# lalithsuresh/rapid

Hardware: NVIDIA H100
Metric: alert_cells_per_sec_to_converged_cut (higher is better)
Workload: dtype u16

## Files before the change

rapid_b200/csrc/cd_bucketed.cu:

```cuda
#include <cooperative_groups.h>

#include <algorithm>
#include <climits>
#include <cstdlib>

#include "cd_internal.cuh"

namespace cg = cooperative_groups;

namespace rapid {

#ifndef RAPID_UNI_MINBLOCKS
#define RAPID_UNI_MINBLOCKS 5
#endif
#ifndef RAPID_SPLIT_LOOP
#define RAPID_SPLIT_LOOP 0
#endif
#ifndef RAPID_PF
#define RAPID_PF 2
#endif
#ifndef RAPID_INVAL_SPLIT
#define RAPID_INVAL_SPLIT 1
#endif
#ifndef RAPID_PF_L1
#define RAPID_PF_L1 0
#endif
#if RAPID_PF_L1
#define RAPID_PF_ASM "prefetch.global.L1 [%0];"
#else
#define RAPID_PF_ASM "prefetch.global.L2 [%0];"
#endif
#ifndef RAPID_MEMO
#define RAPID_MEMO 1
#endif

constexpr int TILE_R = 1024;
constexpr int UNI_THREADS = 128;
constexpr int GEN_THREADS = 256;
constexpr int STAGE = 32;
constexpr int MAXK = RAPID_MAX_K;
constexpr int SMALL_SEG = 4;
constexpr uint32_t T32_NONE = 0xFFFFFFFFu;
constexpr uint64_t T64_NONE = ~0ULL;
constexpr uint32_t RF_K3 = 16u;
constexpr uint32_t RF_ACTIVE = 32u;
constexpr uint32_t RF_MIXED_EMIT = 64u;

constexpr uint32_t MX_ON = 1u, MX_NEG = 2u, MX_HAS_E = 4u, MX_DONE = 8u;
constexpr uint32_t MX_REF = 32u;
constexpr uint32_t MX_TIME = 16u;

constexpr uint32_t PF_SEEN = 1u;
constexpr uint32_t PF_NEGINF = 2u;

struct ChunkAcc {
    uint32_t nL, nH, tp, nUn, fl, minTH, minTLun, pad_;
    uint64_t h1, h2;
    uint32_t nLp, nHp, tpc, minBHp, minBLlong, pad2_;
    uint64_t h1p, h2p;
};

constexpr int PF_SHIFT = 30;
constexpr uint32_t TP_MASK = (1u << PF_SHIFT) - 1u;

struct Partials {
    uint4* cnt;
    uint4* cntp;
    uint64_t* minTH;
    uint64_t* minTLun;
    uint64_t* h1;
    uint64_t* h2;
    uint64_t* h1p;
    uint64_t* h2p;
    uint2* seq;
    int32_t* flag;
    ChunkAcc* chunk;
    int n_tiles;
};

struct Bucketed {
    DevBuf<int32_t> sidx;
    DevBuf<int32_t> seg_cnt, batch_slots;
    DevBuf<int32_t> bins, ovf, cell_batch;
    DevBuf<SubjDesc> desc;
    DevBuf<SubjWalk> walk;
    DevBuf<uint8_t> s_ring, s_status;
    DevBuf<int32_t> p_flag;
    DevBuf<ChunkAcc> p_chunk;
    DevBuf<uint4> p_cnt, p_cntp;
    DevBuf<uint64_t> p_minTH, p_minTLun, p_h1, p_h2, p_h1p, p_h2p;
    DevBuf<uint2> p_seq;
    DevBuf<SubjWalk> pwalk;
    DevBuf<unsigned char> ra_dev;
    DevBuf<uint32_t> mx_fl;
    DevBuf<uint64_t> mx_a, mx_cand, mx_emax;
    DevBuf<uint64_t> mx_p1, mx_p2;
    DevBuf<int32_t> mx_pc;
    DevBuf<unsigned long long> mx_e1, mx_e2;
    DevBuf<int32_t> mx_ec;
    DevBuf<uint64_t> estar;
    DevBuf<int32_t> mx_changed;
    DevBuf<uint32_t> mx_dev;
    DevBuf<int32_t> batch_index;
#if RAPID_INVAL_SPLIT
    DevBuf<int32_t> inv_res, inv_ticket;
    DevBuf<unsigned long long> inv_h1, inv_h2;
#endif
    DevBuf<int32_t> wl_slots, wl_count, wl_listed, wl_so_tab;
    DevBuf<uint8_t> wl_in_tile;
    DevBuf<uint8_t> has_so;
    size_t in_list_slots = 0;
    int n_tiles = 0;
    size_t part_cap = 0;
    int slots_uniform = 0, slots_generic = 0;
    int resolve_grid = 0;
};

struct Visit {
    int c0, c1;
    bool crossL, crossH;
    uint32_t tL, tH;
};

__device__ __forceinline__ Visit visit_uniform(uint32_t ur, const SubjDesc& d, const SubjWalk& w, int L, int H) {
    Visit v;
    v.tL = 0; v.tH = 0;
    if (ur == d.pmask) {
        v.c0 = __popc(ur); v.c1 = __popc(ur | d.bmask);
        v.tL = d.tLf; v.tH = d.tHf;
    } else {
        int c = __popc(ur);
        v.c0 = c;
        const int nr = d.nr;
        for (int q = 0; q < nr; ++q) {
            const int k = w.ring[q];
            const bool isnew = !((ur >> k) & 1u);
            c += isnew;
            if (isnew && c == L) v.tL = w.time[q];
            if (isnew && c == H) v.tH = w.time[q];
        }
        v.c1 = c;
    }
    v.crossL = v.c0 < L && v.c1 >= L;
    v.crossH = v.c0 < H && v.c1 >= H;
    return v;
}

__device__ __forceinline__ Visit visit_counts(uint32_t ur, const SubjDesc& d, uint32_t RM, int L, int H) {
    Visit v;
    v.tL = 0; v.tH = 0;
    v.c0 = __popc(ur);
    v.c1 = __popc((ur | d.bmask) & RM);
    v.crossL = v.c0 < L && v.c1 >= L;
    v.crossH = v.c0 < H && v.c1 >= H;
    return v;
}

struct Acc {
    uint32_t nL = 0, nH = 0, tp = 0, nUn = 0, flags = 0;
    uint32_t minTH = T32_NONE, minTLun = T32_NONE;
    uint64_t h1 = 0, h2 = 0;
    uint32_t nLp = 0, nHp = 0, tpc = 0, minBHp = T32_NONE, minBLlong = T32_NONE;
    uint64_t h1p = 0, h2p = 0;
};

__device__ __forceinline__ bool accumulate(Acc& a, const Visit& v, const SubjDesc& d, int L, int H) {
    if (v.c0 >= L && v.c0 < H) a.tp++;
    if (v.crossL) a.nL++;
    if (v.crossH) { a.nH++; a.minTH = min(a.minTH, v.tH); a.h1 += d.mix1; a.h2 += d.mix2; }
    if (v.c1 >= L && v.c1 < H) {
        if (v.crossL) { a.nUn++; a.minTLun = min(a.minTLun, v.tL); }
        else a.flags |= PF_NEGINF;
        return true;
    }
    return false;
}
// ... 684 lines not shown
    uint64_t* mx_p1;
    uint64_t* mx_p2;
    int32_t* mx_pc;
    uint64_t* estar;
    unsigned long long* mx_e1;
    unsigned long long* mx_e2;
    int32_t* mx_ec;
    int32_t* mx_changed;
    uint32_t* mx_dev;
    const int32_t* slot_of;
    const int32_t* obs;
    const int32_t* touch;
    const int32_t* batch_index;
    int32_t serial;
#if RAPID_INVAL_SPLIT
    int inv_split;
    int32_t* inv_res;
    unsigned long long* inv_h1;
    unsigned long long* inv_h2;
    int32_t* inv_ticket;
#endif
};

__device__ __forceinline__ int32_t block_sum_i32(int32_t v, int32_t* s_red) {
    __syncthreads();
#pragma unroll
    for (int o = 16; o > 0; o >>= 1) v += __shfl_down_sync(0xffffffffu, v, o);
    if ((threadIdx.x & 31) == 0) s_red[threadIdx.x >> 5] = v;
    __syncthreads();
    int32_t s = 0;
    for (int w = 0; w < (int)(blockDim.x >> 5); ++w) s += s_red[w];
    return s;
}

__device__ __forceinline__ void reduce_fresh(const ResolveArgs& a, ChunkAcc* s_fresh, int* s_fhave) {
    const ApplyArgs& ap = a.ap;
    if (threadIdx.x < 32) {
        uint32_t nL = 0, nH = 0, tp = 0, nUn = 0, fl = 0, mTH = T32_NONE, mTL = T32_NONE;
        uint64_t h1 = 0, h2 = 0;
        uint32_t nLp = 0, nHp = 0, tpc = 0, mBH = T32_NONE, mBL = T32_NONE;
        uint64_t h1p = 0, h2p = 0;
        for (int c = threadIdx.x; c < a.n_chunks; c += 32) {
            const ChunkAcc k = ap.part.chunk[c];
            nL += k.nL; nH += k.nH; tp += k.tp; nUn += k.nUn; fl |= k.fl;
            if (k.nH) mTH = min(mTH, k.minTH);
            if (k.nUn) mTL = min(mTL, k.minTLun);
            h1 += k.h1; h2 += k.h2;
            if (a.seq) {
                nLp += k.nLp; nHp += k.nHp; tpc += k.tpc; mBH = min(mBH, k.minBHp); mBL = min(mBL, k.minBLlong);
                h1p += k.h1p; h2p += k.h2p;
            }
        }
#pragma unroll
        for (int o = 16; o > 0; o >>= 1) {
            nL += __shfl_down_sync(0xffffffffu, nL, o); nH += __shfl_down_sync(0xffffffffu, nH, o);
            tp += __shfl_down_sync(0xffffffffu, tp, o);
            nUn += __shfl_down_sync(0xffffffffu, nUn, o); fl |= __shfl_down_sync(0xffffffffu, fl, o);
            mTH = min(mTH, __shfl_down_sync(0xffffffffu, mTH, o)); mTL = min(mTL, __shfl_down_sync(0xffffffffu, mTL, o));
            h1 += __shfl_down_sync(0xffffffffu, h1, o); h2 += __shfl_down_sync(0xffffffffu, h2, o);
            nLp += __shfl_down_sync(0xffffffffu, nLp, o); nHp += __shfl_down_sync(0xffffffffu, nHp, o);
            tpc += __shfl_down_sync(0xffffffffu, tpc, o);
            mBH = min(mBH, __shfl_down_sync(0xffffffffu, mBH, o)); mBL = min(mBL, __shfl_down_sync(0xffffffffu, mBL, o));
            h1p += __shfl_down_sync(0xffffffffu, h1p, o); h2p += __shfl_down_sync(0xffffffffu, h2p, o);
        }
        if (threadIdx.x == 0) {
            ChunkAcc f;
            f.nL = nL; f.nH = nH; f.tp = tp; f.nUn = nUn; f.fl = fl; f.minTH = mTH; f.minTLun = mTL; f.pad_ = 0; f.h1 = h1; f.h2 = h2;
            f.nLp = nLp; f.nHp = nHp; f.tpc = tpc; f.minBHp = mBH; f.minBLlong = mBL; f.pad2_ = 0; f.h1p = h1p; f.h2p = h2p;
            *s_fresh = f;
            *s_fhave = (nH ? 1 : 0) | (nUn ? 2 : 0);
        }
    }
    __syncthreads();
}

__device__ void phase_finalize1(const ResolveArgs& a, int32_t* s_red) {
    const ApplyArgs& ap = a.ap;
    const int any_down = a.bc->any_down;
    __shared__ ChunkAcc s_fresh;
    __shared__ int s_fhave;
    reduce_fresh(a, &s_fresh, &s_fhave);
    int32_t my_mixed = 0, my_times = 0;
    for (int64_t r = (int64_t)blockIdx.x * blockDim.x + threadIdx.x; r < ap.R; r += (int64_t)gridDim.x * blockDim.x) {
        a.mx_fl[r] = 0;
        uint32_t flags = a.rflags[r] & ~(RF_ANN_NOW | RF_K3 | RF_ACTIVE | RF_PRE_DOWN);
        if (flags & RF_SEEN_DOWN) flags |= RF_PRE_DOWN;
        a.out_h1[r] = 0; a.out_h2[r] = 0; a.out_len[r] = 0;
        const bool active = !(flags & RF_ANNOUNCED) && !((ap.dl.flags & RAPID_DELIVERY_BLOCKED) && ap.dl.blocked[r]);
        if (!active) { a.rflags[r] = flags; a.out_ann[r] = (flags & RF_ANNOUNCED) ? 1 : 0; continue; }
        flags |= RF_ACTIVE;
        uint32_t nL = s_fresh.nL, nH = s_fresh.nH, tp = s_fresh.tp, nUn = s_fresh.nUn, fl = s_fresh.fl;
        uint64_t minTH = s_fresh.minTH, minTLun = s_fresh.minTLun, h1 = s_fresh.h1, h2 = s_fresh.h2;
        uint32_t nLp = s_fresh.nLp, nHp = s_fresh.nHp;
        uint64_t h1p = s_fresh.h1p, h2p = s_fresh.h2p;
        bool haveTH = s_fhave & 1, haveTL = (s_fhave & 2) != 0;
        const int tile = (int)(r / TILE_R);
        for (int c0 = 0; c0 < a.n_chunks; c0 += 4) {
            int on[4];
#pragma unroll
            for (int q = 0; q < 4; ++q) on[q] = c0 + q < a.n_chunks ? ap.part.flag[(size_t)(c0 + q) * ap.part.n_tiles + tile] : 0;
            uint4 q4[4], p4[4];
            uint64_t th[4], tl[4], a1[4], a2[4], b1[4], b2[4];
#pragma unroll
            for (int q = 0; q < 4; ++q) {
                if (!on[q]) continue;
                const size_t p = (size_t)(c0 + q) * ap.Rpad + (size_t)r;
                q4[q] = ap.part.cnt[p]; a1[q] = ap.part.h1[p]; a2[q] = ap.part.h2[p];
                if (!a.counts_only) { th[q] = ap.part.minTH[p]; tl[q] = ap.part.minTLun[p]; }
                if (a.seq) { p4[q] = ap.part.cntp[p]; b1[q] = ap.part.h1p[p]; b2[q] = ap.part.h2p[p]; }
            }
#pragma unroll
            for (int q = 0; q < 4; ++q) {
                if (!on[q]) continue;
                const uint32_t cH = q4[q].y, cUn = q4[q].w;
                nL += q4[q].x; nH += cH; tp += q4[q].z & TP_MASK; nUn += cUn; fl |= q4[q].z >> PF_SHIFT;
                if (!a.counts_only) {
                    if (cH && (!haveTH || th[q] < minTH)) { minTH = th[q]; haveTH = true; }
                    if (cUn && (!haveTL || tl[q] < minTLun)) { minTLun = tl[q]; haveTL = true; }
                }
                h1 += a1[q]; h2 += a2[q];
                if (a.seq) { nLp += p4[q].x; nHp += p4[q].y; h1p += b1[q]; h2p += b2[q]; }
            }
        }
        if ((a.uniform || a.counts_only) ? any_down : (fl & PF_SEEN)) flags |= RF_SEEN_DOWN;
        const int32_t npre_old = a.n_pre[r] + (int32_t)nLp - (int32_t)nHp;
        const int32_t npre_new = npre_old + (int32_t)nL - (int32_t)nH;
        const uint64_t p1_old = a.pend_h1[r] + h1p, p2_old = a.pend_h2[r] + h2p;
        const int32_t pc_old = a.pend_cnt[r] + (int32_t)nHp;
        uint64_t ph1 = p1_old + h1, ph2 = p2_old + h2;
        int32_t pc = pc_old + (int32_t)nH;
        const int32_t untouched_pre = npre_old - (int32_t)tp;
        if (nH > 0 && npre_new == 0) {
            a.out_h1[r] = ph1; a.out_h2[r] = ph2; a.out_len[r] = pc;
            ph1 = 0; ph2 = 0; pc = 0;
            flags |= RF_ANNOUNCED | RF_ANN_NOW | RF_RULE_GE_H;
        } else if (nH > 0 && untouched_pre <= 0 && !(fl & PF_NEGINF)) {
            if (a.counts_only) {
                ++my_times;
                a.mx_fl[r] = MX_TIME;
                a.mx_a[r] = T64_NONE; a.mx_cand[r] = T64_NONE; a.mx_emax[r] = 0;
                a.mx_p1[r] = p1_old; a.mx_p2[r] = p2_old; a.mx_pc[r] = pc_old;
            } else if (!(haveTL && minTLun < minTH)) {
                ++my_mixed;
                atomicMin(&a.bc->mx_first, (int32_t)r);
                a.mx_fl[r] = MX_ON;
                a.mx_a[r] = minTLun; a.mx_cand[r] = T64_NONE; a.mx_emax[r] = 0;
                a.mx_p1[r] = p1_old; a.mx_p2[r] = p2_old; a.mx_pc[r] = pc_old;
            }
        }
        if (npre_new > 0 && (flags & RF_SEEN_DOWN)) flags |= RF_K3;
        a.n_pre[r] = npre_new;
        a.pend_h1[r] = ph1; a.pend_h2[r] = ph2; a.pend_cnt[r] = pc;
        a.rflags[r] = flags;
    }
    const int32_t bm = block_sum_i32(my_mixed, s_red), bt = block_sum_i32(my_times, s_red);
    if (threadIdx.x == 0) {
        if (bm) atomicAdd(&a.bc->n_mixed, bm);
        if (bt) atomicAdd(&a.bc->n_times, bt);
    }
}

struct IVisit { int c0, c1; bool crossL, crossH; uint64_t tL, tH; };

__device__ __forceinline__ IVisit interval_visit(const ApplyArgs& a, int uniform, uint32_t ur, const SubjDesc& d, const SubjWalk* w,
                                                 int64_t r, uint64_t rs) {
    IVisit o;
    if (uniform) {
        const Visit v = visit_uniform(ur, d, *w, a.L, a.H);
        o.c0 = v.c0; o.c1 = v.c1; o.crossL = v.crossL; o.crossH = v.crossH; o.tL = v.tL; o.tH = v.tH;
    } else {
        const GVisit v = visit_generic(ur, d, a.sidx, a.s_ring, a.s_status, a.dl, r, rs, a.L, a.H);
        o.c0 = v.c0; o.c1 = v.c1; o.crossL = v.crossL; o.crossH = v.crossH; o.tL = v.tL; o.tH = v.tH;
    }
    return o;
}

struct PassSmem {
    SubjDesc sd[STAGE];
    SubjWalk sw[STAGE];
    const uint8_t* s_old[STAGE];
};

template <int MODE>
__device__ __noinline__ void mixed_pass(const ResolveArgs& m, PassSmem& sm, const int Sb, const int S_before, const int64_t only_r = -1) {
    const ApplyArgs& a = m.ap;
    const int t = threadIdx.x;
    const uint32_t RM = (1u << a.K) - 1u;
    const int L = a.L, H = a.H;
    const int rblocks = (int)(a.Rpad / GEN_THREADS);
    int mchunks = max(1, min((Sb + STAGE - 1) / STAGE, (2 * (int)gridDim.x + rblocks - 1) / rblocks));
    const int mchunk = max(1, (Sb + mchunks - 1) / mchunks);
    mchunks = (Sb + mchunk - 1) / mchunk;
    const int64_t items = (int64_t)rblocks * mchunks;
    for (int64_t wi = blockIdx.x; wi < items; wi += gridDim.x) {
        const int rb = (int)(wi % rblocks), chunk = (int)(wi / rblocks);
        const int64_t r = (int64_t)rb * GEN_THREADS + t;
        const uint32_t fl = r < a.R ? m.mx_fl[r] : 0u;
        const bool on = (only_r < 0 || r == only_r) &&
                        (MODE == 0 ? ((fl & MX_ON) && !(fl & MX_DONE)) : MODE == 1 ? ((fl & MX_DONE) && (fl & MX_HAS_E) && !(fl & MX_REF)) : ((fl & MX_TIME) != 0));
        if (!__syncthreads_or(on ? 1 : 0)) continue;
        const uint64_t ref = on ? (MODE == 0 ? m.mx_a[r] : MODE == 1 ? m.estar[r] : 0ull) : 0ull;
        const uint64_t rs = splitmix64(a.dl.perm_seed + (uint64_t)(a.rbegin + r));
        const int s0 = chunk * mchunk, s1 = min(Sb, s0 + mchunk);
        uint64_t cand = T64_NONE, emax = 0, h1 = 0, h2 = 0, mTH = T64_NONE, mTL = T64_NONE;
        bool neg = false, has_e = false;
        int cnt = 0;
        for (int base = s0; base < s1; base += STAGE) {
            const int n = min(STAGE, s1 - base);
            __syncthreads();
            if (t < n) {
                const SubjDesc d = a.desc[base + t];
// ... 78 lines not shown
        const int32_t oc = a.mx_pc[r] + a.mx_ec[r];
        a.out_h1[r] = o1; a.out_h2[r] = o2; a.out_len[r] = oc;
        a.pend_h1[r] -= o1; a.pend_h2[r] -= o2; a.pend_cnt[r] -= oc;
        a.mx_e1[r] = 0; a.mx_e2[r] = 0; a.mx_ec[r] = 0;
        a.rflags[r] = (a.rflags[r] | RF_ANNOUNCED | RF_ANN_NOW | RF_MIXED_EMIT) & ~RF_RULE_GE_H;
    }
}

__device__ __noinline__ bool emitted_in_batch(const ResolveArgs& e, int32_t s, int64_t r, uint32_t w_new, uint64_t rs) {
    const ApplyArgs& a = e.ap;
    const uint32_t RM = (1u << a.K) - 1u;
    if (e.touch[s] != e.serial) return __popc(w_new & RM) >= a.H && !e.trans.test(s, r);
    const int b = e.batch_index[s];
    const SubjDesc d = a.desc[b];
    const uint32_t old = seq_state(a, d, b, r, (s >= a.bc->S_before ? 0u : a.rows.get(a.rows.alt_lo(s), r)) & RM, true, true);
    if (__popc(old & RM) >= a.H) return true;
    SubjWalk wl;
    if (e.uniform) wl = a.walk[b];
    const IVisit v = interval_visit(a, e.uniform, old & RM, d, &wl, r, rs);
    return v.crossH && v.tH <= e.estar[r];
}

constexpr int INV_STAGE = 128;
struct InvSmem {
    uint8_t* row[INV_STAGE];
    uint64_t mix1[INV_STAGE], mix2[INV_STAGE];
    uint8_t ne[INV_STAGE];
    const uint8_t* e_row[INV_STAGE * MAXK];
    int32_t e_so[INV_STAGE * MAXK];
    uint8_t e_k[INV_STAGE * MAXK];
    uint8_t flag[INV_STAGE];
    uint8_t dense[INV_STAGE];
    int32_t n_dense;
};

template <bool MX>
__device__ void phase_inval_finalize2(const ResolveArgs& e, int mixed, InvSmem& sm, int32_t* s_red) {
    static_assert(TILE_R == 4 * GEN_THREADS, "a thread owns 4 receivers of a tile");
    const ApplyArgs& a = e.ap;
    const uint32_t RM = (1u << a.K) - 1u;
    const int t = threadIdx.x;
    const int n_list = min(*(volatile int32_t*)a.wl.count, a.wl.cap);
    int32_t my_inval = 0;
#if RAPID_INVAL_SPLIT
    const int P = MX ? 1 : max(1, e.inv_split);
    __shared__ int s_fin;
#else
    constexpr int P = 1;
#endif
    for (int tb = blockIdx.x; tb < a.n_tiles * P; tb += gridDim.x) {
        const int tile = P > 1 ? tb % a.n_tiles : tb;
        int lo = 0, hi = n_list;
        if (P > 1) {
            const int per = max(8, (n_list + P - 1) / P);
            lo = min(n_list, (tb / a.n_tiles) * per); hi = min(n_list, lo + per);
        }
        const int64_t rb = (int64_t)tile * TILE_R + (int64_t)t * 4;
        const uint4 rf4 = *reinterpret_cast<const uint4*>(e.rflags + rb);
        uint32_t flags[4] = {rf4.x, rf4.y, rf4.z, rf4.w};
        bool k3[4];
        bool any_k3 = false;
        bool mine[4];
#pragma unroll
        for (int j = 0; j < 4; ++j) {
            mine[j] = rb + j < a.R && (((flags[j] & RF_MIXED_EMIT) != 0 && mixed) == MX);
            k3[j] = mine[j] && (flags[j] & RF_ACTIVE) && (flags[j] & RF_K3);
            any_k3 |= k3[j];
        }
        int32_t res[4] = {0, 0, 0, 0};
        uint64_t kh1[4] = {0, 0, 0, 0}, kh2[4] = {0, 0, 0, 0};
        if (n_list > 0 && __syncthreads_or(any_k3 ? 1 : 0)) {
            for (int base = lo; base < hi; base += INV_STAGE) {
                const int n = min(INV_STAGE, hi - base);
                __syncthreads();
                if (t == 0) sm.n_dense = 0;
                __syncthreads();
                if (t < n) {
                    const int32_t sl = a.wl.slots[base + t];
                    const uint8_t fl = a.wl.in_tile[(size_t)sl * a.wl.n_tiles + tile];
                    sm.flag[t] = fl;
                    sm.row[t] = a.rows.cur_lo(sl);
                    const int32_t subject = a.slot_subject[sl];
                    sm.mix1[t] = fp_mix1(subject); sm.mix2[t] = fp_mix2(subject);
                    int ne = 0;
                    for (int k = 0; k < a.K; ++k) {
                        const int32_t s2 = a.wl.so_tab[(size_t)sl * SO_STRIDE + k];
                        if (s2 < 0) continue;
                        sm.e_row[t * MAXK + ne] = a.rows.cur_lo(s2);
                        sm.e_so[t * MAXK + ne] = s2; sm.e_k[t * MAXK + ne] = (uint8_t)k;
                        ++ne;
                    }
                    sm.ne[t] = (uint8_t)ne;
                    if (fl) sm.dense[atomicAdd(&sm.n_dense, 1)] = (uint8_t)t;
                }
                __syncthreads();
                if (!any_k3) continue;
                const int nd = sm.n_dense;
                for (int g = 0; g < nd; g += 4) {
                    int idx[4];
                    uint2 w2v[4], e0v[4], e1v[4];
#pragma unroll
                    for (int q = 0; q < 4; ++q) {
                        idx[q] = g + q < nd ? (int)sm.dense[g + q] : -1;
                        w2v[q] = make_uint2(0xFFFFFFFFu, 0xFFFFFFFFu); e0v[q] = make_uint2(0u, 0u); e1v[q] = make_uint2(0u, 0u);
                        if (idx[q] < 0) continue;
                        w2v[q] = a.rows.load4(sm.row[idx[q]], rb);
                        const int eb = idx[q] * MAXK, ne = sm.ne[idx[q]];
                        if (ne > 0) e0v[q] = a.rows.load4(sm.e_row[eb], rb);
                        if (ne > 1) e1v[q] = a.rows.load4(sm.e_row[eb + 1], rb);
                    }
#pragma unroll
                    for (int q = 0; q < 4; ++q) {
                        const int i = idx[q];
                        if (i < 0) continue;
                        const int eb = i * MAXK, ee = eb + sm.ne[i];
                        uint32_t w[4];
#pragma unroll
                        for (int j = 0; j < 4; ++j) w[j] = a.rows.word4(w2v[q], j);
                        uint32_t miss[4];
                        uint32_t anymiss = 0;
#pragma unroll
                        for (int j = 0; j < 4; ++j) {
                            const int c = __popc(w[j] & RM);
                            miss[j] = (k3[j] && c >= a.L && c < a.H) ? (~w[j] & RM) : 0u;
                            anymiss |= miss[j];
                        }
                        if (!anymiss) continue;
                        uint32_t implicit[4] = {0u, 0u, 0u, 0u};
                        for (int ei = eb; ei < ee; ++ei) {
                            const int k = sm.e_k[ei];
                            if (!((anymiss >> k) & 1u)) continue;
                            const uint2 o2 = ei == eb ? e0v[q] : ei == eb + 1 ? e1v[q] : a.rows.load4(sm.e_row[ei], rb);
                            uint32_t wo[4];
#pragma unroll
                            for (int j = 0; j < 4; ++j) wo[j] = a.rows.word4(o2, j);
#pragma unroll
                            for (int j = 0; j < 4; ++j) {
                                if (!((miss[j] >> k) & 1u)) continue;
                                if (__popc(wo[j] & RM) < a.L) continue;
                                if (MX) {
                                    const int64_t r = rb + j;
                                    if (emitted_in_batch(e, sm.e_so[ei], r, wo[j], splitmix64(a.dl.perm_seed + (uint64_t)(a.rbegin + r)))) continue;
                                }
                                implicit[j] |= 1u << k;
                            }
                        }
                        bool any = false;
                        uint32_t trans = 0;
#pragma unroll
                        for (int j = 0; j < 4; ++j) {
                            if (!implicit[j]) continue;
                            any = true;
                            w[j] |= implicit[j];
                            const bool raised = __popc(w[j] & RM) >= a.H;
                            if (raised && mixed) trans |= 1u << j;
                            if (raised) { ++res[j]; kh1[j] += sm.mix1[i]; kh2[j] += sm.mix2[i]; }
                        }
                        if (trans) atomicOr(e.trans.word(a.wl.slots[base + i], rb), trans << (rb & 31));
                        if (any) a.rows.store4(sm.row[i], rb, w);
                    }
                }
            }
        }
#if RAPID_INVAL_SPLIT
        if (P > 1) {
#pragma unroll
            for (int j = 0; j < 4; ++j)
                if (res[j] > 0) { atomicAdd(&e.inv_res[rb + j], res[j]); atomicAdd(&e.inv_h1[rb + j], (unsigned long long)kh1[j]); atomicAdd(&e.inv_h2[rb + j], (unsigned long long)kh2[j]); }
            __threadfence();
            __syncthreads();
// ... 88 lines not shown
    __shared__ int s_last;
    __syncthreads();
    if (threadIdx.x == 0) {
        __threadfence();
        s_last = atomicAdd(&a.bc->ticket, 1) == (int)gridDim.x - 1;
    }
    __syncthreads();
    if (!s_last || threadIdx.x != 0) return;
    __threadfence();
    volatile BatchCounts* b = a.bc;
    BatchCounts c;
    c.n_slots = b->n_slots; c.n_valid = b->n_valid; c.n_batch_subj = b->n_batch_subj; c.any_down = b->any_down;
    c.bad_ring = b->bad_ring; c.bad_dst = b->bad_dst; c.n_mixed = b->n_mixed; c.n_inval = b->n_inval; c.S_before = b->S_before;
    c.overflow = b->overflow; c.need_slots = b->need_slots; c.n_times = b->n_times; c.mixed_iters = b->mixed_iters;
    c.n_pairs = *(volatile int32_t*)a.ap.wl.count; c.ticket = 0; c.serial = serial;
    c.seq_last = b->seq_last; c.seq_down = b->seq_down; c.seq_abort = b->seq_abort; c.seq_a1 = b->seq_a1; c.seq_a2 = b->seq_a2;
    c.mx_first = b->mx_first; c.mx_left = b->mx_left;
    if (c.seq_abort) { c.n_slots = c.S_before; b->n_slots = c.S_before; }
    c.sticky_bad_ring = b->sticky_bad_ring | (c.bad_ring >= 0 ? 1 : 0);
    c.sticky_bad_dst = b->sticky_bad_dst | (c.bad_dst >= 0 ? 1 : 0);
    c.sticky_overflow = b->sticky_overflow | (c.overflow ? 1 : 0);
    b->sticky_bad_ring = c.sticky_bad_ring; b->sticky_bad_dst = c.sticky_bad_dst; b->sticky_overflow = c.sticky_overflow;
    *a.snap = c;
    b->n_valid = 0; b->n_batch_subj = 0; b->any_down = 0; b->bad_ring = -1; b->bad_dst = -1; b->n_mixed = 0; b->n_inval = 0;
    b->overflow = 0; b->need_slots = 0; b->n_times = 0; b->mixed_iters = 0; b->ticket = 0;
    b->seq_last = 0; b->seq_down = INT_MAX; b->seq_abort = 0; b->seq_a1 = 0; b->seq_a2 = 0; b->mx_first = INT_MAX; b->mx_left = 0;
    b->S_before = c.n_slots;
}

__device__ void phase_ref_compare(const ResolveArgs& e, const int64_t r0, const int Sb, const int S_before) {
    static_assert(TILE_R == 4 * GEN_THREADS, "a thread owns 4 receivers of a tile");
    const ApplyArgs& a = e.ap;
    const uint32_t RM = (1u << a.K) - 1u;
    const int t = threadIdx.x;
    constexpr int CH = 64;
    __shared__ const uint8_t* s_row[CH];
    __shared__ uint32_t s_ref[CH];
    const int nch = (Sb + CH - 1) / CH;
    const int64_t items = (int64_t)a.n_tiles * nch;
    for (int64_t wi = blockIdx.x; wi < items; wi += gridDim.x) {
        const int tile = (int)(wi % a.n_tiles), ch = (int)(wi / a.n_tiles);
        const int64_t rb = (int64_t)tile * TILE_R + (int64_t)t * 4;
        const int b0 = ch * CH, nb = min(Sb, b0 + CH) - b0;
        __syncthreads();
        if (t < nb) {
            const int32_t slot = a.desc[b0 + t].slot;
            const uint8_t* row = slot >= S_before ? nullptr : a.rows.cur_lo(slot);
            s_row[t] = row;
            s_ref[t] = row ? a.rows.get(row, r0) & RM : 0u;
        }
        __syncthreads();
        uint32_t bits = 0;
#pragma unroll 8
        for (int i = 0; i < nb; ++i) {
            const uint8_t* row = s_row[i];
            if (row == nullptr) continue;
            const uint2 g = a.rows.load4(row, rb);
#pragma unroll
            for (int j = 0; j < 4; ++j) bits |= ((a.rows.word4(g, j) ^ s_ref[i]) & RM) ? 1u << j : 0u;
        }
        if (bits) atomicOr(&e.mx_dev[rb >> 5], bits << (rb & 31));
    }
}
__device__ void phase_ref_adopt(const ResolveArgs& a, const int64_t r0, int32_t* s_red) {
    const uint32_t f0 = a.mx_fl[r0];
    int32_t my = 0;
    for (int64_t r = (int64_t)blockIdx.x * blockDim.x + threadIdx.x; r < a.ap.R; r += (int64_t)gridDim.x * blockDim.x) {
        const uint32_t fl = a.mx_fl[r];
        const bool dev = (a.mx_dev[r >> 5] >> (r & 31)) & 1u;
        if (r != r0 && (fl & MX_ON) && !(fl & MX_DONE)) {
            if (!dev) {
                a.mx_fl[r] = f0 ? (f0 | MX_REF) : 0u;
                if ((f0 & MX_DONE) && (f0 & MX_HAS_E)) { a.estar[r] = a.estar[r0]; a.mx_e1[r] = a.mx_e1[r0]; a.mx_e2[r] = a.mx_e2[r0]; a.mx_ec[r] = a.mx_ec[r0]; }
            } else {
                ++my;
            }
        }
    }
    const int32_t b = block_sum_i32(my, s_red);
    if (threadIdx.x == 0 && b) atomicAdd(&a.bc->mx_left, b);
    if (blockIdx.x == 0 && threadIdx.x == 0 && f0) a.mx_fl[r0] = f0 | MX_REF;
}

__global__ void __launch_bounds__(GEN_THREADS) k_seq_check(const ResolveArgs* __restrict__ ga) {
    const ResolveArgs& a = *ga;
    const ApplyArgs& ap = a.ap;
    __shared__ int32_t s_red[GEN_THREADS / 32];
    __shared__ ChunkAcc s_fresh;
    __shared__ int s_fhave;
    if (a.bc->overflow) return;
    const int64_t r = (int64_t)blockIdx.x * GEN_THREADS + threadIdx.x;
    const uint32_t rf = r < ap.R ? a.rflags[r] : RF_ANNOUNCED;
    const bool active = r < ap.R && !(rf & RF_ANNOUNCED) && !((ap.dl.flags & RAPID_DELIVERY_BLOCKED) && ap.dl.blocked[r]);
    int32_t bad = 0;
    if (blockIdx.y == 0) {
        reduce_fresh(a, &s_fresh, &s_fhave);
        if (active) {
            uint32_t tpc = s_fresh.tpc, mBH = s_fresh.minBHp, mBL = s_fresh.minBLlong;
            const int tile = (int)(r / TILE_R);
            for (int c = 0; c < a.n_chunks; ++c) {
                if (!ap.part.flag[(size_t)c * ap.part.n_tiles + tile]) continue;
                const size_t p = (size_t)c * ap.Rpad + (size_t)r;
                tpc += ap.part.cntp[p].z;
                const uint2 q = ap.part.seq[p];
                mBH = min(mBH, q.x); mBL = min(mBL, q.y);
            }
            const bool ok = mBH == T32_NONE || (a.n_pre[r] - (int32_t)tpc) > 0 || mBL < mBH;
            if (!ok) bad = 1;
        }
    } else {
        const int32_t S = a.bc->n_slots, S_before = a.bc->S_before;
        const uint32_t last = (uint32_t)a.bc->seq_last;
        const int nchunks = (int)gridDim.y - 1;
        const int per = (S + nchunks - 1) / nchunks;
        const int32_t q0 = min(S, ((int)blockIdx.y - 1) * per), q1 = min(S, q0 + per);
        const uint32_t RM = (1u << ap.K) - 1u;
        const uint32_t bDown = receiver_down_batch(ap, rf, false);
        for (int32_t sl = q0; sl < q1; ++sl) {
            if (sl >= S_before || !ap.wl.has_so[sl] || a.touch[sl] == a.serial) continue;
            if (!active || bDown == T32_NONE) continue;
            const uint32_t us = ap.rows.get(sl, r) & RM;
            const int cs = __popc(us);
            if (cs < ap.L || cs >= ap.H) continue;
            for (int k = 0; k < ap.K; ++k) {
                const int32_t so = ap.wl.so_tab[(size_t)sl * SO_STRIDE + k];
                if (so < 0 || ((us >> k) & 1u)) continue;
                const bool o_touched = a.touch[so] == a.serial;
                const int bo_idx = o_touched ? a.batch_index[so] : 0;
                const uint32_t uo = so < S_before ? (ap.rows.get(so, r) & RM) : 0u;
                const uint32_t bLo = observer_L_batch(uo, o_touched ? &ap.desc[bo_idx] : nullptr, o_touched ? &ap.pwalk[bo_idx] : nullptr, ap.L);
                if (bLo != T32_NONE && max(bLo, bDown) <= last) bad = 1;
            }
        }
    }
    const int32_t b = block_sum_i32(bad, s_red);
    if (threadIdx.x == 0 && b) { atomicAdd(&a.bc->seq_abort, b); atomicAdd(blockIdx.y == 0 ? &a.bc->seq_a1 : &a.bc->seq_a2, b); }
}

__global__ void __launch_bounds__(GEN_THREADS) k_finalize1(const ResolveArgs* __restrict__ ga) {
    const ResolveArgs& a = *ga;
    __shared__ int32_t s_red[GEN_THREADS / 32];
    if (a.bc->overflow || a.bc->seq_abort) return;
    phase_finalize1(a, s_red);
}

__global__ void __launch_bounds__(GEN_THREADS, 2) k_mixed_flip(const ResolveArgs* __restrict__ ga) {
    const ResolveArgs& a = *ga;
    cg::grid_group grid = cg::this_grid();
    __shared__ PassSmem sm;
    __shared__ int32_t s_red[GEN_THREADS / 32];
    if (a.bc->overflow || a.bc->seq_abort) return;
    const int Sb = a.bc->n_batch_subj, S_before = a.bc->S_before;
    if (a.counts_only && a.bc->n_times > 0 && Sb > 0) {
        mixed_pass<2>(a, sm, Sb, S_before);
        grid.sync();
        phase_classify_moments(a, s_red);
        grid.sync();
    }
    const int mixed = *(volatile int32_t*)&a.bc->n_mixed > 0 ? 1 : 0;
    if (mixed && Sb > 0) {
        auto analyse = [&](const int64_t only_r) -> int {
            int it = 0;
            for (;; ++it) {
                mixed_pass<0>(a, sm, Sb, S_before, only_r);
                grid.sync();
                if (blockIdx.x == 0 && threadIdx.x == 0) a.mx_changed[(it + 2) & 3] = 0;
                phase_mixed_update(a, &a.mx_changed[it & 3], s_red, only_r);
                grid.sync();
                if (*(volatile int32_t*)&a.mx_changed[it & 3] == 0 || it > Sb + 1) break;
            }
            mixed_pass<1>(a, sm, Sb, S_before, only_r);
            grid.sync();
            if (blockIdx.x == 0 && threadIdx.x == 0) { a.mx_changed[0] = 0; a.mx_changed[1] = 0; a.mx_changed[2] = 0; a.mx_changed[3] = 0; }
            grid.sync();
            return it + 1;
        };
        int iters = 0;
        int left = 1;
        if (a.uniform && !a.ap.seq) {
            const int64_t r0 = (int64_t)*(volatile int32_t*)&a.bc->mx_first;
            iters = analyse(r0);
            phase_ref_compare(a, r0, Sb, S_before);
            grid.sync();
            phase_ref_adopt(a, r0, s_red);
            grid.sync();
            left = *(volatile int32_t*)&a.bc->mx_left;
            for (int64_t q = (int64_t)blockIdx.x * blockDim.x + threadIdx.x; q < (int64_t)(a.ap.Rpad >> 5); q += (int64_t)gridDim.x * blockDim.x) a.mx_dev[q] = 0;
        }
        if (left > 0) iters += analyse(-1);
        if (blockIdx.x == 0 && threadIdx.x == 0) a.bc->mixed_iters = iters;
        phase_mixed_commit(a);
        grid.sync();
    }
    for (int b = blockIdx.x * blockDim.x + threadIdx.x; b < Sb; b += gridDim.x * blockDim.x) a.cur_w[a.ap.desc[b].slot] ^= 1;
}

__global__ void __launch_bounds__(GEN_THREADS, 2) k_inval_finalize2(const ResolveArgs* __restrict__ ga) {
    const ResolveArgs& a = *ga;
    __shared__ InvSmem sm;
    __shared__ int32_t s_red[GEN_THREADS / 32];
    const int mixed = a.bc->n_mixed > 0 ? 1 : 0;
    if (!a.bc->overflow && !a.bc->seq_abort) phase_inval_finalize2<false>(a, mixed, sm, s_red);
    if (a.bc->seq_abort) {
        const int32_t s0 = a.bc->S_before, s1 = a.bc->n_slots;
        for (int32_t sl = s0 + blockIdx.x * blockDim.x + threadIdx.x; sl < s1; sl += gridDim.x * blockDim.x)
            const_cast<int32_t*>(a.slot_of)[a.ap.slot_subject[sl]] = -1;
    }
    if (!mixed) resolve_tail(a, a.serial);
}

__global__ void __launch_bounds__(GEN_THREADS, 2) k_marks(const ResolveArgs* __restrict__ ga) {
    const ResolveArgs& a = *ga;
    cg::grid_group grid = cg::this_grid();
    __shared__ InvSmem sm;
    __shared__ int32_t s_red[GEN_THREADS / 32];
    if (a.bc->n_mixed <= 0) return;
    phase_inval_finalize2<true>(a, 1, sm, s_red);
    grid.sync();
    if (*(volatile int32_t*)&a.bc->n_inval > 0) {
        phase_mixed_mark(a, *(volatile int32_t*)&a.bc->n_slots);
        grid.sync();
    }
    phase_inval_unmark(a);
    resolve_tail(a, a.serial);
}

static Bucketed* state(CD* cd) {
    if (!cd->bucketed_state) cd->bucketed_state = new Bucketed();
    return static_cast<Bucketed*>(cd->bucketed_state);
}

void bucketed_destroy(CD* cd) {
    if (cd->bucketed_state) { delete static_cast<Bucketed*>(cd->bucketed_state); cd->bucketed_state = nullptr; }
}

static WorkList worklist(const Bucketed* b) {
    WorkList wl;
    wl.has_so = b->has_so.p; wl.so_tab = b->wl_so_tab.p; wl.in_tile = b->wl_in_tile.p; wl.listed = b->wl_listed.p;
    wl.slots = b->wl_slots.p; wl.count = b->wl_count.p;
    wl.cap = (int32_t)std::min<size_t>(b->in_list_slots, 0x7fffffff); wl.n_tiles = b->n_tiles;
    return wl;
}

template <typename T>
static int32_t grow_keep(DevBuf<T>& buf, size_t n_old, size_t n_new, cudaStream_t s) {
    DevBuf<T> nb;
    RAPID_CHECK(nb.reserve(std::max<size_t>(n_new, 1)));
    RAPID_CUDA(cudaMemsetAsync(nb.p, 0, std::max<size_t>(n_new, 1) * sizeof(T), s));
    if (n_old && buf.p) RAPID_CUDA(cudaMemcpyAsync(nb.p, buf.p, n_old * sizeof(T), cudaMemcpyDeviceToDevice, s));
    RAPID_CUDA(cudaStreamSynchronize(s));
    std::swap(buf.p, nb.p); std::swap(buf.cap, nb.cap);
    return RAPID_OK;
}

static int32_t ensure_pre_capacity(CD* cd, Bucketed* b) {
    const size_t slots = cd->S_cap;
    if (slots <= b->in_list_slots) return RAPID_OK;
    const size_t o = b->in_list_slots, nt = (size_t)b->n_tiles;
    RAPID_CHECK(grow_keep(b->wl_in_tile, o * nt, slots * nt, cd->stream));
    RAPID_CHECK(grow_keep(b->wl_listed, o, slots, cd->stream));
    RAPID_CHECK(grow_keep(b->wl_slots, o, slots, cd->stream));
    RAPID_CHECK(grow_keep(b->wl_so_tab, o * SO_STRIDE, slots * SO_STRIDE, cd->stream));
    RAPID_CHECK(grow_keep(b->has_so, o, slots, cd->stream));
    b->in_list_slots = slots;
    return RAPID_OK;
}

int32_t bucketed_prep_buffers(CD* cd, int64_t A, PrepOut* po) {
    Bucketed* b = state(cd);
    b->n_tiles = (int)(cd->Rpad / TILE_R);
    RAPID_CHECK(ensure_pre_capacity(cd, b));
    const size_t a = (size_t)std::max<int64_t>(A, 1);
    RAPID_CHECK(b->desc.reserve(a)); RAPID_CHECK(b->walk.reserve(a)); RAPID_CHECK(b->pwalk.reserve(a));
    RAPID_CHECK(b->sidx.reserve(a)); RAPID_CHECK(b->s_ring.reserve(a)); RAPID_CHECK(b->s_status.reserve(a));
    const size_t slots = std::max<size_t>(cd->S_cap, 1);
    RAPID_CHECK(b->batch_index.reserve(slots));
    RAPID_CHECK(b->batch_slots.reserve(slots));
    RAPID_CHECK(b->bins.reserve(slots * 64));
    RAPID_CHECK(b->ovf.reserve(a)); RAPID_CHECK(b->cell_batch.reserve(a));
    if (slots > b->seg_cnt.cap) {
        RAPID_CHECK(b->seg_cnt.reserve(slots));
        RAPID_CUDA(cudaMemsetAsync(b->seg_cnt.p, 0, b->seg_cnt.cap * sizeof(int32_t), cd->stream));
    }
    po->desc = b->desc.p; po->walk = b->walk.p; po->sidx = b->sidx.p; po->s_ring = b->s_ring.p; po->s_status = b->s_status.p;
    po->batch_index = b->batch_index.p; po->seg_cnt = b->seg_cnt.p; po->batch_slots = b->batch_slots.p;
    po->bins = b->bins.p; po->ovf = b->ovf.p; po->pwalk = b->pwalk.p; po->cell_batch = b->cell_batch.p;
    po->wl = worklist(b);
    return RAPID_OK;
}

__global__ void k_clear_sticky(BatchCounts* bc) { bc->sticky_bad_ring = 0; bc->sticky_bad_dst = 0; bc->sticky_overflow = 0; }

int32_t bucketed_clear_sticky(CD* cd) {
    k_clear_sticky<<<1, 1, 0, cd->stream>>>(cd->counts.p);
    RAPID_KERNEL_CHECK();
// ... 121 lines not shown
            const double f = w - std::floor(w);
            double eff;
            if (w <= 1.0) eff = 0.85 + 0.15 * w;
            else eff = w / (std::floor(w) + (f > 0 ? std::max(f, 0.6) : 0.0));
            eff -= 0.001 * cc;
            if (eff > best) { best = eff; n_chunks = cc; }
        }
        if (const char* ov = getenv("RAPID_B200_CHUNKS")) n_chunks = std::max(1, std::min(Sb, atoi(ov)));
    }
    cd->last_chunks = n_chunks;
    const size_t pn = (size_t)n_chunks * cd->Rpad;
    RAPID_CHECK(b->p_cnt.reserve(pn)); RAPID_CHECK(b->p_minTH.reserve(pn)); RAPID_CHECK(b->p_minTLun.reserve(pn));
    RAPID_CHECK(b->p_h1.reserve(pn)); RAPID_CHECK(b->p_h2.reserve(pn));
    if (seq) {
        RAPID_CHECK(b->p_cntp.reserve(pn)); RAPID_CHECK(b->p_h1p.reserve(pn)); RAPID_CHECK(b->p_h2p.reserve(pn));
        RAPID_CHECK(b->p_seq.reserve(pn));
    }
    RAPID_CHECK(b->mx_fl.reserve(cd->Rpad)); RAPID_CHECK(b->mx_a.reserve(cd->Rpad)); RAPID_CHECK(b->mx_cand.reserve(cd->Rpad));
    RAPID_CHECK(b->mx_emax.reserve(cd->Rpad)); RAPID_CHECK(b->mx_p1.reserve(cd->Rpad)); RAPID_CHECK(b->mx_p2.reserve(cd->Rpad));
    RAPID_CHECK(b->mx_pc.reserve(cd->Rpad)); RAPID_CHECK(b->estar.reserve(cd->Rpad));
    if (!b->mx_dev.p || b->mx_dev.cap < (cd->Rpad >> 5)) {
        RAPID_CHECK(b->mx_dev.reserve(std::max<size_t>(cd->Rpad >> 5, 1)));
        RAPID_CUDA(cudaMemsetAsync(b->mx_dev.p, 0, std::max<size_t>(cd->Rpad >> 5, 1) * sizeof(uint32_t), s));
    }
    if (!b->mx_e1.p) {
        RAPID_CHECK(b->mx_e1.reserve(cd->Rpad)); RAPID_CHECK(b->mx_e2.reserve(cd->Rpad)); RAPID_CHECK(b->mx_ec.reserve(cd->Rpad));
        RAPID_CUDA(cudaMemsetAsync(b->mx_e1.p, 0, cd->Rpad * sizeof(unsigned long long), s));
        RAPID_CUDA(cudaMemsetAsync(b->mx_e2.p, 0, cd->Rpad * sizeof(unsigned long long), s));
        RAPID_CUDA(cudaMemsetAsync(b->mx_ec.p, 0, cd->Rpad * sizeof(int32_t), s));
    }
    RAPID_CHECK(b->p_flag.reserve((size_t)n_chunks * std::max(b->n_tiles, 1)));
    RAPID_CHECK(b->p_chunk.reserve((size_t)n_chunks));
    Partials part{b->p_cnt.p, b->p_cntp.p, b->p_minTH.p, b->p_minTLun.p, b->p_h1.p, b->p_h2.p, b->p_h1p.p, b->p_h2p.p, b->p_seq.p, b->p_flag.p, b->p_chunk.p, b->n_tiles};

    ApplyArgs ap;
    ap.rows = RowRef{cd->masks.p, cd->cur.p, cd->Rpad, cd->row_stride, cd->nbuf, cd->hb}; ap.Rpad = cd->Rpad;
    ap.K = cd->K; ap.H = cd->H; ap.L = cd->L; ap.R = cd->R; ap.rbegin = cd->rbegin;
    ap.rflags = cd->rflags.p; ap.dl = dl; ap.bc = cd->counts.p;
    ap.desc = b->desc.p; ap.walk = b->walk.p; ap.pwalk = b->pwalk.p; ap.slot_subject = cd->slot_subject.p;
    ap.touch = cd->touch.p; ap.batch_index = b->batch_index.p; ap.serial = cd->batch_serial; ap.seq = seq ? 1 : 0;
    ap.sidx = b->sidx.p; ap.s_ring = b->s_ring.p; ap.s_status = b->s_status.p;
    ap.part = part; ap.n_tiles = b->n_tiles; ap.wl = worklist(b);

    RAPID_CUDA(cudaEventRecord(cd->evk0, s));
    if (swar) {
        dim3 grid((unsigned)b->n_tiles, (unsigned)n_chunks);
        if (cd->hb == 2) launch_uniform<2>(grid, s, ap, counts_only, seq);
        else launch_uniform<8>(grid, s, ap, counts_only, seq);
        cd->last_path = counts_only ? 4 : 2;
    } else {
        dim3 grid((unsigned)(cd->Rpad / GEN_THREADS), (unsigned)n_chunks);
        k_apply_generic<<<grid, GEN_THREADS, 0, s>>>(ap);
        cd->last_path = 3;
    }
    RAPID_KERNEL_CHECK();
    RAPID_CUDA(cudaEventRecord(cd->evk1, s));

    ResolveArgs ra;
    ra.ap = ap; ra.bc = cd->counts.p;
    ra.emit = MarkPlane{cd->emit_marks.p, cd->Rpad / 32}; ra.trans = MarkPlane{cd->trans_marks.p, cd->Rpad / 32}; ra.snap = cd->counts_snap.p; ra.n_chunks = n_chunks;
    ra.uniform = uniform ? 1 : 0; ra.counts_only = counts_only ? 1 : 0; ra.cur_w = cd->cur.p;
    ra.seq = seq ? 1 : 0; ra.seq_dev = nullptr;
    ra.n_pre = cd->n_pre.p; ra.rflags = cd->rflags.p; ra.pend_h1 = cd->pend_h1.p; ra.pend_h2 = cd->pend_h2.p;
    ra.pend_cnt = cd->pend_cnt.p; ra.out_h1 = cd->out_h1.p; ra.out_h2 = cd->out_h2.p; ra.out_len = cd->out_len.p; ra.out_ann = cd->out_ann.p;
    ra.mx_fl = b->mx_fl.p; ra.mx_a = b->mx_a.p; ra.mx_cand = b->mx_cand.p; ra.mx_emax = b->mx_emax.p;
    ra.mx_p1 = b->mx_p1.p; ra.mx_p2 = b->mx_p2.p; ra.mx_pc = b->mx_pc.p; ra.estar = b->estar.p;
    ra.mx_e1 = b->mx_e1.p; ra.mx_e2 = b->mx_e2.p; ra.mx_ec = b->mx_ec.p; ra.mx_changed = b->mx_changed.p; ra.mx_dev = b->mx_dev.p;
    ra.slot_of = cd->slot_of.p; ra.obs = cd->view->obs.p; ra.touch = cd->touch.p; ra.batch_index = b->batch_index.p;
    ra.serial = cd->batch_serial;
#if RAPID_INVAL_SPLIT
    const int inv_split = b->n_tiles >= 64 ? 1 : std::min(32, (2 * TARGET_SMS + std::max(b->n_tiles, 1) - 1) / std::max(b->n_tiles, 1));
    if (inv_split > 1 && !b->inv_res.p) {
        RAPID_CHECK(b->inv_res.reserve(cd->Rpad)); RAPID_CHECK(b->inv_h1.reserve(cd->Rpad)); RAPID_CHECK(b->inv_h2.reserve(cd->Rpad));
        RAPID_CHECK(b->inv_ticket.reserve((size_t)std::max(b->n_tiles, 1)));
        RAPID_CUDA(cudaMemsetAsync(b->inv_res.p, 0, cd->Rpad * sizeof(int32_t), s));
        RAPID_CUDA(cudaMemsetAsync(b->inv_h1.p, 0, cd->Rpad * sizeof(unsigned long long), s));
        RAPID_CUDA(cudaMemsetAsync(b->inv_h2.p, 0, cd->Rpad * sizeof(unsigned long long), s));
        RAPID_CUDA(cudaMemsetAsync(b->inv_ticket.p, 0, (size_t)std::max(b->n_tiles, 1) * sizeof(int32_t), s));
    }
    ra.inv_split = inv_split; ra.inv_res = b->inv_res.p; ra.inv_h1 = b->inv_h1.p; ra.inv_h2 = b->inv_h2.p; ra.inv_ticket = b->inv_ticket.p;
#endif
    const unsigned rblocks = (unsigned)(cd->Rpad / GEN_THREADS);
    const int cgrid = std::max(1, std::min(b->resolve_grid, std::max(32, 4 * (int)rblocks)));
    RAPID_CHECK(b->ra_dev.reserve(sizeof(ResolveArgs)));
    RAPID_CUDA(cudaMemcpyAsync(b->ra_dev.p, &ra, sizeof(ResolveArgs), cudaMemcpyHostToDevice, s));
    const ResolveArgs* ga = (const ResolveArgs*)b->ra_dev.p;
    void* args[] = {(void*)&ga};
    if (seq) {
        const unsigned echunks = (unsigned)std::max<int64_t>(1, std::min<int64_t>(64, 32 * TARGET_SMS / std::max(1u, rblocks)));
        k_seq_check<<<dim3(rblocks, 1 + echunks), GEN_THREADS, 0, s>>>(ga);
        RAPID_KERNEL_CHECK();
        cd->last_launches += 1;
    }
    k_finalize1<<<rblocks, GEN_THREADS, 0, s>>>(ga);
    RAPID_KERNEL_CHECK();
    RAPID_CUDA(cudaLaunchCooperativeKernel((void*)k_mixed_flip, dim3((unsigned)cgrid), dim3(GEN_THREADS), args, 0, s));
#if RAPID_INVAL_SPLIT
    k_inval_finalize2<<<(unsigned)(std::max(b->n_tiles, 1) * inv_split), GEN_THREADS, 0, s>>>(ga);
#else
    k_inval_finalize2<<<(unsigned)std::max(b->n_tiles, 1), GEN_THREADS, 0, s>>>(ga);
#endif
    RAPID_KERNEL_CHECK();
    RAPID_CUDA(cudaLaunchCooperativeKernel((void*)k_marks, dim3((unsigned)cgrid), dim3(GEN_THREADS), args, 0, s));
    cd->last_launches += 5;
    RAPID_CUDA(cudaMemcpyAsync(cd->h_counts.p, cd->counts_snap.p, sizeof(BatchCounts), cudaMemcpyDeviceToHost, s));
    return RAPID_OK;
}

}
```

Measured before the change: 21.08 million.

## Pass resolve args as grid constants, cap finalize grid, vectorize observer loads

Resolve kernels now take ResolveArgs by value as a __grid_constant__ parameter, which removes the per-batch host-to-device memcpy of the argument struct and the device buffer that held it. k_finalize1 is launched with a grid capped at twice the resolve grid and relies on its grid-stride loop. The per-row loads in finalize1 are hoisted to the top of the loop body. The observer-table row in inval finalize is read with 128-bit loads into a fully unrolled MAXK loop. A profiling script is also added. The risks are the larger kernel parameter block and less parallelism in finalize1 when R is large.

```diff
diff --git a/profiles/epoch_breakdown.py b/profiles/epoch_breakdown.py
--- /dev/null
+++ b/profiles/epoch_breakdown.py
@@ -0,0 +1,108 @@
+import argparse
+import json
+import os
+import sys
+
+import numpy as np
+
+ROOT = os.path.dirname(os.path.dirname(os.path.abspath(__file__)))
+sys.path.insert(0, ROOT)
+
+import bench
+
+
+def main():
+    ap = argparse.ArgumentParser()
+    ap.add_argument("--workload", default="c5", choices=["c5", "c3", "c2"])
+    ap.add_argument("--nodes", type=int, default=0)
+    ap.add_argument("--emulate-shard", type=int, default=0, help="rank 0's shard of a G-way run on one GPU")
+    ap.add_argument("--epochs", type=int, default=3)
+    ap.add_argument("--out", default=None)
+    args = ap.parse_args()
+    if args.nodes <= 0:
+        args.nodes = bench.DEFAULT_NODES[args.workload]
+    out = args.out or os.path.join(ROOT, "profiles", "h100", "epoch_breakdown_%s%s.json" % (
+        args.workload, "_shard%d" % args.emulate_shard if args.emulate_shard > 1 else ""))
+
+    import torch
+    from torch.profiler import ProfilerActivity, profile
+    import rapid_b200 as rb
+    from rapid_b200 import workloads as W
+
+    K, H, L = bench.K, bench.H, bench.L
+    n, nj = args.nodes, bench.n_joiners(args)
+    hb, off, ports = W.packed_endpoints(0, n + nj)
+    view = rb.MembershipView.from_packed(K, hb[: off[n]], off[: n + 1], ports[:n])
+    if nj:
+        import ctypes as C
+        from rapid_b200 import _native as N
+        jh = hb[off[n]: off[n + nj]]
+        first = C.c_int32(0)
+        N.check(N.lib().rapid_view_register_joiners(view._h, nj, N.ptr(np.ascontiguousarray(jh)),
+                                                    N.ptr(np.ascontiguousarray(off[n:] - off[n])),
+                                                    N.ptr(np.ascontiguousarray(ports[n:])), C.byref(first)))
+    obs, _ = view.tables()
+    ring0 = view.getRing(0)
+    joiner_obs = view.joinerTables() if nj else np.zeros((0, K), np.int32)
+    st = bench.Stream(args, W, obs, joiner_obs, ring0)
+    assert len(st.batches) == 1, "one-batch workloads only (the asynchronous epoch)"
+    hi, lo = W.node_ids(0, n)
+    cfg = view.getCurrentConfigurationId(hi, lo)
+    Gs = max(1, args.emulate_shard)
+    R = n // Gs
+    blocked = W.blocked_by_receiver(st.blocked, ring0, 0, R)
+    cl = rb.VirtualCluster(view, H, L, n_receivers=R, receiver_begin=0, max_subjects=st.subjects + 64)
+    fp = rb.FastPaxos(cfg, n, sender_capacity=n)
+    b = st.batches[0]
+    d_dst, d_ring, d_status = (torch.from_numpy(x).cuda() for x in (b.dst, b.ring, b.status))
+    d_blocked = torch.from_numpy(blocked).cuda()
+
+    def epoch():
+        fp.epochAsync(cl, cfg, st.cells[0], d_dst.data_ptr(), d_ring.data_ptr(), d_status.data_ptr(),
+                      blocked_dev=d_blocked.data_ptr(), perm_seed=st.perm[0])
+        return fp.result()
+
+    for _ in range(5):
+        epoch()
+    torch.cuda.synchronize()
+    with profile(activities=[ProfilerActivity.CPU, ProfilerActivity.CUDA]) as prof:
+        for i in range(args.epochs):
+            torch.cuda.synchronize()
+            with torch.profiler.record_function("epoch%d" % i):
+                epoch()
+            torch.cuda.synchronize()
+
+    evs = [e for e in prof.events() if e.device_type == torch.autograd.DeviceType.CUDA and not e.name.startswith("epoch")]
+    cpu_epochs = sorted([e for e in prof.events() if e.name.startswith("epoch")], key=lambda e: e.time_range.start)
+    t_last = cpu_epochs[-1].time_range.start
+    evs = sorted([e for e in evs if e.time_range.start >= t_last], key=lambda e: e.time_range.start)
+    rows, prev_end, t0 = [], None, evs[0].time_range.start
+    for e in evs:
+        s, d = e.time_range.start, e.time_range.end - e.time_range.start
+        gap = 0.0 if prev_end is None else max(0.0, s - prev_end)
+        rows.append({"name": e.name[:120], "start_us": round(s - t0, 2), "dur_us": round(d, 2), "gap_before_us": round(gap, 2)})
+        prev_end = max(prev_end or 0, e.time_range.end)
+    span = prev_end - t0
+    busy = sum(r["dur_us"] for r in rows)
+    props = torch.cuda.get_device_properties(0)
+    try:
+        import subprocess
+        q = subprocess.run(["nvidia-smi", "--query-gpu=name,power.limit,clocks.max.sm", "--format=csv,noheader"],
+                           capture_output=True, text=True, timeout=30).stdout.strip().splitlines()[0]
+    except Exception as ex:
+        q = "nvidia-smi failed: %r" % (ex,)
+    res = {"workload": st.name(args, 0), "receivers": R, "emulate_shard": Gs, "gpu": props.name, "nvidia_smi": q,
+           "how": "torch.profiler (CUDA activities) over %d epochs after 5 warm-up ones, last epoch shown; each epoch is "
+                  "FastPaxos.epochAsync + result(), as in bench.py's timed loop" % args.epochs,
+           "epoch_device_span_us": round(span, 2), "busy_us": round(busy, 2), "idle_us": round(span - busy, 2),
+           "events": rows}
+    os.makedirs(os.path.dirname(out), exist_ok=True)
+    with open(out, "w") as f:
+        json.dump(res, f, indent=1)
+    for r in rows:
+        print("%10.1f %9.1f %8.1f  %s" % (r["start_us"], r["dur_us"], r["gap_before_us"], r["name"]), file=sys.stderr)
+    print("span %.1f us, busy %.1f us, idle %.1f us -> %s" % (span, busy, span - busy, out), file=sys.stderr)
+
+
+if __name__ == "__main__":
+    main()
diff --git a/rapid_b200/csrc/cd_bucketed.cu b/rapid_b200/csrc/cd_bucketed.cu
--- a/rapid_b200/csrc/cd_bucketed.cu
+++ b/rapid_b200/csrc/cd_bucketed.cu
@@ -91,7 +91,6 @@
     DevBuf<uint64_t> p_minTH, p_minTLun, p_h1, p_h2, p_h1p, p_h2p;
     DevBuf<uint2> p_seq;
     DevBuf<SubjWalk> pwalk;
-    DevBuf<unsigned char> ra_dev;
     DevBuf<uint32_t> mx_fl;
     DevBuf<uint64_t> mx_a, mx_cand, mx_emax;
     DevBuf<uint64_t> mx_p1, mx_p2;
@@ -942,11 +941,15 @@
     reduce_fresh(a, &s_fresh, &s_fhave);
     int32_t my_mixed = 0, my_times = 0;
     for (int64_t r = (int64_t)blockIdx.x * blockDim.x + threadIdx.x; r < ap.R; r += (int64_t)gridDim.x * blockDim.x) {
+        const uint32_t rf0 = a.rflags[r];
+        const bool blocked = (ap.dl.flags & RAPID_DELIVERY_BLOCKED) && ap.dl.blocked[r];
+        const int32_t npre0 = a.n_pre[r], pc0 = a.pend_cnt[r];
+        const uint64_t ph10 = a.pend_h1[r], ph20 = a.pend_h2[r];
         a.mx_fl[r] = 0;
-        uint32_t flags = a.rflags[r] & ~(RF_ANN_NOW | RF_K3 | RF_ACTIVE | RF_PRE_DOWN);
+        uint32_t flags = rf0 & ~(RF_ANN_NOW | RF_K3 | RF_ACTIVE | RF_PRE_DOWN);
         if (flags & RF_SEEN_DOWN) flags |= RF_PRE_DOWN;
         a.out_h1[r] = 0; a.out_h2[r] = 0; a.out_len[r] = 0;
-        const bool active = !(flags & RF_ANNOUNCED) && !((ap.dl.flags & RAPID_DELIVERY_BLOCKED) && ap.dl.blocked[r]);
+        const bool active = !(flags & RF_ANNOUNCED) && !blocked;
         if (!active) { a.rflags[r] = flags; a.out_ann[r] = (flags & RF_ANNOUNCED) ? 1 : 0; continue; }
         flags |= RF_ACTIVE;
         uint32_t nL = s_fresh.nL, nH = s_fresh.nH, tp = s_fresh.tp, nUn = s_fresh.nUn, fl = s_fresh.fl;
@@ -983,10 +986,10 @@
             }
         }
         if ((a.uniform || a.counts_only) ? any_down : (fl & PF_SEEN)) flags |= RF_SEEN_DOWN;
-        const int32_t npre_old = a.n_pre[r] + (int32_t)nLp - (int32_t)nHp;
+        const int32_t npre_old = npre0 + (int32_t)nLp - (int32_t)nHp;
         const int32_t npre_new = npre_old + (int32_t)nL - (int32_t)nH;
-        const uint64_t p1_old = a.pend_h1[r] + h1p, p2_old = a.pend_h2[r] + h2p;
-        const int32_t pc_old = a.pend_cnt[r] + (int32_t)nHp;
+        const uint64_t p1_old = ph10 + h1p, p2_old = ph20 + h2p;
+        const int32_t pc_old = pc0 + (int32_t)nHp;
         uint64_t ph1 = p1_old + h1, ph2 = p2_old + h2;
         int32_t pc = pc_old + (int32_t)nH;
         const int32_t untouched_pre = npre_old - (int32_t)tp;
@@ -1231,10 +1234,19 @@
                     sm.row[t] = a.rows.cur_lo(sl);
                     const int32_t subject = a.slot_subject[sl];
                     sm.mix1[t] = fp_mix1(subject); sm.mix2[t] = fp_mix2(subject);
+                    static_assert(SO_STRIDE == 16 && MAXK <= SO_STRIDE, "one 64-byte row of the observer table");
+                    int32_t so[SO_STRIDE];
+                    const int4* so4 = reinterpret_cast<const int4*>(a.wl.so_tab + (size_t)sl * SO_STRIDE);
+#pragma unroll
+                    for (int v = 0; v < SO_STRIDE / 4; ++v) {
+                        const int4 x = so4[v];
+                        so[4 * v] = x.x; so[4 * v + 1] = x.y; so[4 * v + 2] = x.z; so[4 * v + 3] = x.w;
+                    }
                     int ne = 0;
-                    for (int k = 0; k < a.K; ++k) {
-                        const int32_t s2 = a.wl.so_tab[(size_t)sl * SO_STRIDE + k];
-                        if (s2 < 0) continue;
+#pragma unroll
+                    for (int k = 0; k < MAXK; ++k) {
+                        const int32_t s2 = so[k];
+                        if (k >= a.K || s2 < 0) continue;
                         sm.e_row[t * MAXK + ne] = a.rows.cur_lo(s2);
                         sm.e_so[t * MAXK + ne] = s2; sm.e_k[t * MAXK + ne] = (uint8_t)k;
                         ++ne;
@@ -1489,8 +1501,7 @@
     if (blockIdx.x == 0 && threadIdx.x == 0 && f0) a.mx_fl[r0] = f0 | MX_REF;
 }
 
-__global__ void __launch_bounds__(GEN_THREADS) k_seq_check(const ResolveArgs* __restrict__ ga) {
-    const ResolveArgs& a = *ga;
+__global__ void __launch_bounds__(GEN_THREADS) k_seq_check(const __grid_constant__ ResolveArgs a) {
     const ApplyArgs& ap = a.ap;
     __shared__ int32_t s_red[GEN_THREADS / 32];
     __shared__ ChunkAcc s_fresh;
@@ -1544,15 +1555,13 @@
     if (threadIdx.x == 0 && b) { atomicAdd(&a.bc->seq_abort, b); atomicAdd(blockIdx.y == 0 ? &a.bc->seq_a1 : &a.bc->seq_a2, b); }
 }
 
-__global__ void __launch_bounds__(GEN_THREADS) k_finalize1(const ResolveArgs* __restrict__ ga) {
-    const ResolveArgs& a = *ga;
+__global__ void __launch_bounds__(GEN_THREADS) k_finalize1(const __grid_constant__ ResolveArgs a) {
     __shared__ int32_t s_red[GEN_THREADS / 32];
     if (a.bc->overflow || a.bc->seq_abort) return;
     phase_finalize1(a, s_red);
 }
 
-__global__ void __launch_bounds__(GEN_THREADS, 2) k_mixed_flip(const ResolveArgs* __restrict__ ga) {
-    const ResolveArgs& a = *ga;
+__global__ void __launch_bounds__(GEN_THREADS, 2) k_mixed_flip(const __grid_constant__ ResolveArgs a) {
     cg::grid_group grid = cg::this_grid();
     __shared__ PassSmem sm;
     __shared__ int32_t s_red[GEN_THREADS / 32];
@@ -1602,8 +1611,7 @@
     for (int b = blockIdx.x * blockDim.x + threadIdx.x; b < Sb; b += gridDim.x * blockDim.x) a.cur_w[a.ap.desc[b].slot] ^= 1;
 }
 
-__global__ void __launch_bounds__(GEN_THREADS, 2) k_inval_finalize2(const ResolveArgs* __restrict__ ga) {
-    const ResolveArgs& a = *ga;
+__global__ void __launch_bounds__(GEN_THREADS, 2) k_inval_finalize2(const __grid_constant__ ResolveArgs a) {
     __shared__ InvSmem sm;
     __shared__ int32_t s_red[GEN_THREADS / 32];
     const int mixed = a.bc->n_mixed > 0 ? 1 : 0;
@@ -1616,8 +1624,7 @@
     if (!mixed) resolve_tail(a, a.serial);
 }
 
-__global__ void __launch_bounds__(GEN_THREADS, 2) k_marks(const ResolveArgs* __restrict__ ga) {
-    const ResolveArgs& a = *ga;
+__global__ void __launch_bounds__(GEN_THREADS, 2) k_marks(const __grid_constant__ ResolveArgs a) {
     cg::grid_group grid = cg::this_grid();
     __shared__ InvSmem sm;
     __shared__ int32_t s_red[GEN_THREADS / 32];
@@ -1905,23 +1912,20 @@
 #endif
     const unsigned rblocks = (unsigned)(cd->Rpad / GEN_THREADS);
     const int cgrid = std::max(1, std::min(b->resolve_grid, std::max(32, 4 * (int)rblocks)));
-    RAPID_CHECK(b->ra_dev.reserve(sizeof(ResolveArgs)));
-    RAPID_CUDA(cudaMemcpyAsync(b->ra_dev.p, &ra, sizeof(ResolveArgs), cudaMemcpyHostToDevice, s));
-    const ResolveArgs* ga = (const ResolveArgs*)b->ra_dev.p;
-    void* args[] = {(void*)&ga};
+    void* args[] = {(void*)&ra};
     if (seq) {
         const unsigned echunks = (unsigned)std::max<int64_t>(1, std::min<int64_t>(64, 32 * TARGET_SMS / std::max(1u, rblocks)));
-        k_seq_check<<<dim3(rblocks, 1 + echunks), GEN_THREADS, 0, s>>>(ga);
+        k_seq_check<<<dim3(rblocks, 1 + echunks), GEN_THREADS, 0, s>>>(ra);
         RAPID_KERNEL_CHECK();
         cd->last_launches += 1;
     }
-    k_finalize1<<<rblocks, GEN_THREADS, 0, s>>>(ga);
+    k_finalize1<<<std::min(rblocks, 2u * (unsigned)b->resolve_grid), GEN_THREADS, 0, s>>>(ra);
     RAPID_KERNEL_CHECK();
     RAPID_CUDA(cudaLaunchCooperativeKernel((void*)k_mixed_flip, dim3((unsigned)cgrid), dim3(GEN_THREADS), args, 0, s));
 #if RAPID_INVAL_SPLIT
-    k_inval_finalize2<<<(unsigned)(std::max(b->n_tiles, 1) * inv_split), GEN_THREADS, 0, s>>>(ga);
+    k_inval_finalize2<<<(unsigned)(std::max(b->n_tiles, 1) * inv_split), GEN_THREADS, 0, s>>>(ra);
 #else
-    k_inval_finalize2<<<(unsigned)std::max(b->n_tiles, 1), GEN_THREADS, 0, s>>>(ga);
+    k_inval_finalize2<<<(unsigned)std::max(b->n_tiles, 1), GEN_THREADS, 0, s>>>(ra);
 #endif
     RAPID_KERNEL_CHECK();
     RAPID_CUDA(cudaLaunchCooperativeKernel((void*)k_marks, dim3((unsigned)cgrid), dim3(GEN_THREADS), args, 0, s));
```

Result: faster. 21.48 million (median of 6 runs) (+1.9%).
